# infraheads/tvidz

Hardware: AMD Instinct MI355X
Metric: 1080p frames/sec scene-cut scoring (luma SAD + select), frames resident in HBM (higher is better)
Workload: dtype u8

## Files before the change

include/tvz.h:

```cpp
#ifndef TVZ_H
#define TVZ_H

#include <stddef.h>
#include <stdint.h>

#ifdef __cplusplus
extern "C" {
#endif

#define TVZ_VERSION 403

typedef enum tvz_status {
    TVZ_OK = 0,
    TVZ_ERR_INVALID = -1,
    TVZ_ERR_HIP = -2,
    TVZ_ERR_NOMEM = -3,
    TVZ_ERR_UNSUPPORTED = -4,
    TVZ_ERR_WORKSPACE = -5,
    TVZ_ERR_COMM = -6
} tvz_status;

#define TVZ_KTH_NEVER 0x7fffffff

int tvz_version(void);
const char *tvz_last_error(void);


size_t tvz_scene_workspace_bytes(int64_t T, int32_t H, int32_t W);

size_t tvz_scene_state_bytes(int32_t H, int32_t W, int32_t bytes_per_sample);
int tvz_scene_state_reset(void *d_state, void *hip_stream);

#define TVZ_SHAPE_AUTO 0u
#define TVZ_SHAPE_NO_NT (1u << 30)
#define TVZ_SHAPE(U, tc) ((uint32_t)(U) | ((uint32_t)(tc) << 8))

int tvz_luma_sad_u8(const uint8_t *d_luma, int64_t T, int32_t H, int32_t W,
                    int64_t frame_stride_bytes, int64_t row_stride_bytes,
                    uint64_t *d_sad_out, void *d_workspace, size_t workspace_bytes,
                    void *hip_stream);

int tvz_scene_select(const uint64_t *d_sad, int64_t T, int32_t H, int32_t W,
                     int32_t bitdepth, double threshold, const double *d_prev_mafd,
                     uint8_t *d_selected, double *d_score, double *d_mafd, void *hip_stream);

int tvz_scene_scores_u8(const uint8_t *d_luma, int64_t T, int32_t H, int32_t W,
                        int64_t frame_stride_bytes, int64_t row_stride_bytes, void *d_state,
                        int32_t bitdepth, double threshold, uint64_t *d_sad_out, double *d_mafd,
                        double *d_score, uint8_t *d_selected, int32_t *d_cuts, int32_t cuts_cap,
                        void *d_workspace, size_t workspace_bytes, uint32_t shape,
                        void *hip_stream);

int tvz_scene_scores_u16(const uint16_t *d_luma, int64_t T, int32_t H, int32_t W,
                         int64_t frame_stride_bytes, int64_t row_stride_bytes, void *d_state,
                         int32_t bitdepth, double threshold, uint64_t *d_sad_out, double *d_mafd,
                         double *d_score, uint8_t *d_selected, int32_t *d_cuts, int32_t cuts_cap,
                         void *d_workspace, size_t workspace_bytes, uint32_t shape,
                         void *hip_stream);

typedef struct tvz_corpus tvz_corpus;

int tvz_corpus_create(tvz_corpus **out, int device);
int tvz_corpus_destroy(tvz_corpus *c);

int tvz_corpus_reserve(tvz_corpus *c, int64_t n_rows, int64_t n_keys);

int tvz_corpus_upload(tvz_corpus *c, const int32_t *h_video_ids, const int64_t *h_offsets,
                      const double *h_keys, int64_t n_rows, int64_t n_keys);

int tvz_corpus_upsert(tvz_corpus *c, int32_t video_id, const double *h_keys, int64_t n);

int tvz_corpus_clear(tvz_corpus *c);

int tvz_corpus_stats(tvz_corpus *c, int64_t *n_rows, int64_t *n_keys, int64_t *arena_keys);

int tvz_corpus_build_index(tvz_corpus *c);
int tvz_corpus_index_stats(tvz_corpus *c, int64_t *n_indexed_rows, int64_t *n_delta_rows,
                           int64_t *n_postings, int64_t *n_distinct_keys, int64_t *n_builds);
int tvz_corpus_bucket_stats(tvz_corpus *c, int64_t out[6]);


#define TVZ_ALGO_AUTO 0
#define TVZ_ALGO_Q1 1
#define TVZ_ALGO_TILE 2
#define TVZ_ALGO_JOIN 3
#define TVZ_ALGO_INDEX 4
#define TVZ_ALGO_PAIR 0x100
#define TVZ_ALGO_NO_PAIR 0x200
#define TVZ_ALGO_WAVE 0x400
#define TVZ_ALGO_NO_WAVE 0x800
#define TVZ_ALGO_PREFER_WAVE 0x1000

size_t tvz_match_workspace_bytes(int32_t Q, int32_t max_query_len, int32_t cap, int32_t k,
                                 int32_t n_ranks);
size_t tvz_match_workspace_bytes_long(int32_t Q, int32_t max_query_len, int32_t cap, int32_t k,
                                      int32_t n_ranks, int64_t total_query_keys);

int tvz_match(tvz_corpus *c, const double *d_queries, const int64_t *d_q_offsets,
              int32_t Q, int32_t max_query_len, int32_t min_match,
              const int32_t *d_exclude_ids, int32_t cap,
              int32_t *d_hits, int32_t *d_hits_n, void *d_workspace, size_t workspace_bytes,
              int32_t algo, void *hip_stream);

int tvz_match_topk(tvz_corpus *c, const double *d_queries, const int64_t *d_q_offsets,
                   int32_t Q, int32_t max_query_len, int32_t min_match,
                   const int32_t *d_exclude_ids, int32_t cap, int32_t k, int32_t *d_out,
                   void *d_workspace, size_t workspace_bytes, int32_t algo, void *hip_stream);

int tvz_find_duplicates(tvz_corpus *c, const double *h_query, int64_t n, int32_t min_match,
                        int32_t exclude_id, int64_t cap, int32_t *h_out_ids,
                        int32_t *h_out_counts, int32_t *h_out_kth, int64_t *n_out);

int tvz_topk(const int32_t *d_lists, const int32_t *d_lists_n, int32_t n_lists, int32_t Q,
             int32_t cap, int32_t k, int32_t *d_topk, void *hip_stream);

int tvz_topk_shard(const int32_t *d_hits, const int32_t *d_hits_n, int32_t Q, int32_t cap,
                   int32_t k, int32_t *d_out, void *hip_stream);
int tvz_match_topk_shards(tvz_corpus *const *shards, int32_t n_shards, const double *d_queries,
                          const int64_t *d_q_offsets, int32_t Q, int32_t max_query_len, int32_t min_match,
                          const int32_t *d_exclude_ids, int32_t cap, int32_t k, int32_t *d_blocks,
                          int32_t *d_topk, int32_t *d_totals, void *d_workspace, size_t workspace_bytes,
                          int32_t algo, void *hip_stream);
int tvz_topk_merge(const int32_t *d_gathered, int32_t n_ranks, int32_t Q, int32_t k,
                   int32_t *d_topk, int32_t *d_totals, void *hip_stream);

#define TVZ_UNIQUE_ID_BYTES 128
typedef struct tvz_comm tvz_comm;

int tvz_comm_unique_id(void *out_id );
int tvz_comm_init(tvz_comm **out, const void *unique_id, int32_t n_ranks, int32_t rank,
                  int32_t device);
int tvz_comm_info(tvz_comm *comm, int32_t *n_ranks, int32_t *rank);
int tvz_comm_destroy(tvz_comm *comm);

int tvz_match_sharded(tvz_corpus *c, tvz_comm *comm, const double *d_queries,
                      const int64_t *d_q_offsets, int32_t Q, int32_t max_query_len,
                      int32_t min_match, const int32_t *d_exclude_ids, int32_t cap, int32_t k,
                      int32_t *d_topk, int32_t *d_totals, void *d_workspace,
                      size_t workspace_bytes, int32_t algo, void *hip_stream);

int tvz_align(tvz_corpus *c, const double *d_query, int32_t n, double eps, double max_offset,
              int32_t *d_out, int64_t out_rows, int64_t *n_rows, void *hip_stream);


int tvz_find_duplicates_tol(tvz_corpus *c, const double *h_query, int64_t n, double tol,
                            int32_t min_match, int32_t exclude_id, int64_t cap, int32_t *h_out_ids,
                            int32_t *h_out_counts, int32_t *h_out_kth, int64_t *n_out);
size_t tvz_match_tol_workspace_bytes(int32_t Q, int32_t max_query_len, int64_t total_query_keys);
int tvz_match_tol(tvz_corpus *c, const double *d_queries, const int64_t *d_q_offsets, int32_t Q,
                  int32_t max_query_len, double tol, int32_t min_match, const int32_t *d_exclude_ids,
                  int32_t cap, int32_t *d_hits, int32_t *d_hits_n, void *d_workspace,
                  size_t workspace_bytes, void *hip_stream);

size_t tvz_match_tol_topk_workspace_bytes(int32_t Q, int32_t max_query_len, int64_t total_query_keys,
                                          int32_t k, int32_t n_ranks);
int tvz_match_tol_topk(tvz_corpus *c, const double *d_queries, const int64_t *d_q_offsets, int32_t Q,
                       int32_t max_query_len, double tol, int32_t min_match, const int32_t *d_exclude_ids,
                       int32_t k, int32_t *d_out, void *d_workspace, size_t workspace_bytes,
                       void *hip_stream);
int tvz_match_tol_sharded(tvz_corpus *c, tvz_comm *comm, const double *d_queries, const int64_t *d_q_offsets,
                          int32_t Q, int32_t max_query_len, double tol, int32_t min_match,
                          const int32_t *d_exclude_ids, int32_t k, int32_t *d_topk, int32_t *d_totals,
                          void *d_workspace, size_t workspace_bytes, void *hip_stream);


int tvz_read_records(int fd, int64_t file_offset, int64_t n_records, int64_t record_bytes,
                     const void *magic, int64_t header_bytes, int64_t payload_bytes, void *h_dst,
                     int64_t *n_done);

int tvz_read_stream(int fd, int64_t n_records, int64_t payload_bytes, int64_t skip_bytes, void *h_dst,
                    int64_t *n_done);

#ifdef __cplusplus
}
#endif
#endif
```

profiles/microbatch_scene.py:

```python
#!/usr/bin/env python3
import json
import os
import sys
import time

import numpy as np
import torch

sys.path.insert(0, os.path.dirname(os.path.dirname(os.path.abspath(__file__))))
from tvidz_amd import _lib, scene

H, W = (int(sys.argv[1]), int(sys.argv[2])) if len(sys.argv) > 2 else (1080, 1920)
dev = torch.device("cuda:0")
lib = _lib.load()
big = torch.randint(0, 256, (2048, H, W), dtype=torch.uint8, device=dev)
for T in (32, 64, 128, 256, 512, 1024, 2048):
    frames = big[:T]
    res = {}
    variants = [("auto", (0, 0, 1))] + [(f"U{u}tc{tc}", (u, tc, 1)) for u in (1, 2, 4, 8) for tc in (8, 16, 32, 64, 128, 256)]
    for name, tune in variants:
        sc = scene.SceneScorer(H, W, T, dev)
        ts = []
        for r in range(30):
            a, b = torch.cuda.Event(enable_timing=True), torch.cuda.Event(enable_timing=True)
            a.record(); sc.score_batch(frames, carry=False, shape=_lib.shape(*tune)); b.record()
            torch.cuda.synchronize()
            ts.append(a.elapsed_time(b))
        res[name] = round(float(np.median(ts[5:])) * 1e3, 1)
    best = min(res, key=res.get)
    print(json.dumps({"T": T, "auto_us": res["auto"], "best": best, "best_us": res[best],
                      "best_GBps": round((T - 1) * H * W / res[best] / 1e3, 1),
                      "top": sorted(res.items(), key=lambda kv: kv[1])[:5]}))

T = 256
host = [torch.randint(0, 256, (T, H, W), dtype=torch.uint8).pin_memory() for _ in range(2)]
devb = [torch.empty((T, H, W), dtype=torch.uint8, device=dev) for _ in range(2)]
sc = scene.SceneScorer(H, W, T, dev)
copy_s = torch.cuda.Stream()
n_batches = 40
torch.cuda.synchronize()
t0 = time.perf_counter()
evs = [None, None]
for i in range(n_batches):
    s = i & 1
    with torch.cuda.stream(copy_s):
        if evs[s] is not None:
            copy_s.wait_event(evs[s])
        devb[s].copy_(host[s], non_blocking=True)
        ce = torch.cuda.Event(); ce.record(copy_s)
    torch.cuda.current_stream().wait_event(ce)
    sc.score_batch(devb[s], carry=False)
    evs[s] = torch.cuda.Event(); evs[s].record()
torch.cuda.synchronize()
dt = time.perf_counter() - t0
print(json.dumps({"pcie_inclusive_fps": round(n_batches * T / dt), "GBps_h2d": round(n_batches * T * H * W / dt / 1e9, 1),
                  "batch": T, "note": "pinned host luma -> H2D -> score, double buffered"}))
```

profiles/tune_scene.py:

```python
#!/usr/bin/env python3
import itertools
import json
import os
import sys

import numpy as np
import torch

sys.path.insert(0, os.path.dirname(os.path.dirname(os.path.abspath(__file__))))
from tvidz_amd import _lib, scene

T = int(sys.argv[1]) if len(sys.argv) > 1 else 10000
ROUNDS = int(sys.argv[2]) if len(sys.argv) > 2 else 7
H, W = 1080, 1920
dev = torch.device("cuda:0")
lib = _lib.load()
frames = torch.randint(0, 256, (T, H, W), dtype=torch.uint8, device=dev)
if len(sys.argv) > 3 and sys.argv[3] == "tc":
    variants = [(8, tc, 1) for tc in (128, 192, 256, 320, 384, 448, 512, 640, 832, 1280, 2560)]
else:
    variants = [(U, tc, nt) for U, tc, nt in itertools.product((1, 2, 4, 8), (64, 128, 256, 512), (0, 1))]
sc = scene.SceneScorer(H, W, T, dev)
times = {v: [] for v in variants}
ref = None
for r in range(ROUNDS):
    for v in variants:
        a, b = torch.cuda.Event(enable_timing=True), torch.cuda.Event(enable_timing=True)
        a.record()
        sad, _, _, _ = sc.score_batch(frames, carry=False, shape=_lib.shape(*v))
        b.record()
        torch.cuda.synchronize()
        if r == 0:
            s = sad.clone()
            if ref is None:
                ref = s
            assert torch.equal(ref, s), v
        else:
            times[v].append(a.elapsed_time(b))
rows = []
for v, t in times.items():
    med, mn = float(np.median(t)), float(np.min(t))
    rows.append({"U": v[0], "tc": v[1], "nt": v[2], "median_ms": round(med, 4), "min_ms": round(mn, 4),
                 "GBps_median": round((T - 1) * H * W / med / 1e6, 1)})
rows.sort(key=lambda r: r["median_ms"])
for r in rows:
    print(json.dumps(r))
```

tvidz_amd/_lib.py:

```python
from __future__ import annotations

import ctypes as C
import os
import threading

_HERE = os.path.dirname(os.path.abspath(__file__))
SO_PATH = os.environ.get("TVZ_LIB") or os.path.join(_HERE, "libtvz.so")

KTH_NEVER = 0x7FFFFFFF
VERSION = 403

_P = C.c_void_p
SIGNATURES = {
    "tvz_version": (C.c_int, []),
    "tvz_last_error": (C.c_char_p, []),
    "tvz_scene_workspace_bytes": (C.c_size_t, [C.c_int64, C.c_int32, C.c_int32]),
    "tvz_scene_state_bytes": (C.c_size_t, [C.c_int32, C.c_int32, C.c_int32]),
    "tvz_scene_state_reset": (C.c_int, [_P, _P]),
    "tvz_luma_sad_u8": (C.c_int, [_P, C.c_int64, C.c_int32, C.c_int32, C.c_int64, C.c_int64,
                                  _P, _P, C.c_size_t, _P]),
    "tvz_scene_select": (C.c_int, [_P, C.c_int64, C.c_int32, C.c_int32, C.c_int32, C.c_double, _P,
                                   _P, _P, _P, _P]),
    "tvz_scene_scores_u8": (C.c_int, [_P, C.c_int64, C.c_int32, C.c_int32, C.c_int64, C.c_int64, _P,
                                      C.c_int32, C.c_double, _P, _P, _P, _P, _P, C.c_int32, _P,
                                      C.c_size_t, C.c_uint32, _P]),
    "tvz_scene_scores_u16": (C.c_int, [_P, C.c_int64, C.c_int32, C.c_int32, C.c_int64, C.c_int64, _P,
                                       C.c_int32, C.c_double, _P, _P, _P, _P, _P, C.c_int32, _P,
                                       C.c_size_t, C.c_uint32, _P]),
    "tvz_corpus_create": (C.c_int, [C.POINTER(C.c_void_p), C.c_int]),
    "tvz_corpus_destroy": (C.c_int, [_P]),
    "tvz_corpus_reserve": (C.c_int, [_P, C.c_int64, C.c_int64]),
    "tvz_corpus_upload": (C.c_int, [_P, _P, _P, _P, C.c_int64, C.c_int64]),
    "tvz_corpus_upsert": (C.c_int, [_P, C.c_int32, _P, C.c_int64]),
    "tvz_corpus_clear": (C.c_int, [_P]),
    "tvz_corpus_build_index": (C.c_int, [_P]),
    "tvz_corpus_index_stats": (C.c_int, [_P] + [C.POINTER(C.c_int64)] * 5),
    "tvz_corpus_bucket_stats": (C.c_int, [_P, C.POINTER(C.c_int64)]),
    "tvz_corpus_stats": (C.c_int, [_P, C.POINTER(C.c_int64), C.POINTER(C.c_int64),
                                   C.POINTER(C.c_int64)]),
    "tvz_match_workspace_bytes": (C.c_size_t, [C.c_int32, C.c_int32, C.c_int32, C.c_int32, C.c_int32]),
    "tvz_match_workspace_bytes_long": (C.c_size_t, [C.c_int32, C.c_int32, C.c_int32, C.c_int32, C.c_int32, C.c_int64]),
    "tvz_match": (C.c_int, [_P, _P, _P, C.c_int32, C.c_int32, C.c_int32, _P, C.c_int32, _P, _P, _P,
                            C.c_size_t, C.c_int32, _P]),
    "tvz_match_topk": (C.c_int, [_P, _P, _P, C.c_int32, C.c_int32, C.c_int32, _P, C.c_int32, C.c_int32,
                                 _P, _P, C.c_size_t, C.c_int32, _P]),
    "tvz_find_duplicates": (C.c_int, [_P, _P, C.c_int64, C.c_int32, C.c_int32, C.c_int64, _P, _P, _P,
                                      C.POINTER(C.c_int64)]),
    "tvz_topk": (C.c_int, [_P, _P, C.c_int32, C.c_int32, C.c_int32, C.c_int32, _P, _P]),
    "tvz_topk_shard": (C.c_int, [_P, _P, C.c_int32, C.c_int32, C.c_int32, _P, _P]),
    "tvz_topk_merge": (C.c_int, [_P, C.c_int32, C.c_int32, C.c_int32, _P, _P, _P]),
    "tvz_match_topk_shards": (C.c_int, [_P, C.c_int32, _P, _P, C.c_int32, C.c_int32, C.c_int32, _P, C.c_int32,
                                        C.c_int32, _P, _P, _P, _P, C.c_size_t, C.c_int32, _P]),
    "tvz_comm_unique_id": (C.c_int, [_P]),
    "tvz_comm_init": (C.c_int, [C.POINTER(C.c_void_p), _P, C.c_int32, C.c_int32, C.c_int32]),
    "tvz_comm_info": (C.c_int, [_P, C.POINTER(C.c_int32), C.POINTER(C.c_int32)]),
    "tvz_comm_destroy": (C.c_int, [_P]),
    "tvz_match_sharded": (C.c_int, [_P, _P, _P, _P, C.c_int32, C.c_int32, C.c_int32, _P, C.c_int32,
                                    C.c_int32, _P, _P, _P, C.c_size_t, C.c_int32, _P]),
    "tvz_find_duplicates_tol": (C.c_int, [_P, _P, C.c_int64, C.c_double, C.c_int32, C.c_int32, C.c_int64, _P, _P, _P,
                                          C.POINTER(C.c_int64)]),
    "tvz_match_tol_workspace_bytes": (C.c_size_t, [C.c_int32, C.c_int32, C.c_int64]),
    "tvz_match_tol": (C.c_int, [_P, _P, _P, C.c_int32, C.c_int32, C.c_double, C.c_int32, _P, C.c_int32, _P, _P, _P,
                                C.c_size_t, _P]),
    "tvz_match_tol_topk_workspace_bytes": (C.c_size_t, [C.c_int32, C.c_int32, C.c_int64, C.c_int32, C.c_int32]),
    "tvz_match_tol_topk": (C.c_int, [_P, _P, _P, C.c_int32, C.c_int32, C.c_double, C.c_int32, _P, C.c_int32, _P, _P,
                                     C.c_size_t, _P]),
    "tvz_match_tol_sharded": (C.c_int, [_P, _P, _P, _P, C.c_int32, C.c_int32, C.c_double, C.c_int32, _P, C.c_int32,
                                        _P, _P, _P, C.c_size_t, _P]),
    "tvz_align": (C.c_int, [_P, _P, C.c_int32, C.c_double, C.c_double, _P, C.c_int64, C.POINTER(C.c_int64), _P]),
    "tvz_read_records": (C.c_int, [C.c_int, C.c_int64, C.c_int64, C.c_int64, _P, C.c_int64, C.c_int64, _P,
                                   C.POINTER(C.c_int64)]),
    "tvz_read_stream": (C.c_int, [C.c_int, C.c_int64, C.c_int64, C.c_int64, _P, C.POINTER(C.c_int64)]),
}

ALGO_AUTO, ALGO_Q1, ALGO_TILE, ALGO_JOIN, ALGO_INDEX = 0, 1, 2, 3, 4
ALGO_PAIR, ALGO_NO_PAIR = 0x100, 0x200
ALGO_WAVE, ALGO_NO_WAVE = 0x400, 0x800
ALGO_PREFER_WAVE = 0x1000
SHAPE_AUTO = 0
SHAPE_NO_NT = 1 << 30
UNIQUE_ID_BYTES = 128


def shape(U: int = 0, tc: int = 0, nt: bool = True) -> int:
    s = (int(U) & 0xFF) | (int(tc) << 8)
    if not nt:
        s |= SHAPE_NO_NT
    return s


_lock = threading.Lock()
_lib = None


def _preload_torch_hip_runtime() -> None:
    import torch
    cand = os.path.join(os.path.dirname(torch.__file__), "lib", "libamdhip64.so")
    if os.path.exists(cand):
        C.CDLL(cand, mode=C.RTLD_GLOBAL)


def load() -> C.CDLL:
    global _lib
    if _lib is not None:
        return _lib
    with _lock:
        if _lib is None:
            if not os.path.exists(SO_PATH):
                raise RuntimeError(
                    f"{SO_PATH} is missing: the HIP extension is not built and there is no CPU "
                    "fallback. Run `python -m tvidz_amd.build` (needs hipcc).")
            _preload_torch_hip_runtime()
            lib = C.CDLL(SO_PATH)
            lib.tvz_version.restype, lib.tvz_version.argtypes = C.c_int, []
            if lib.tvz_version() == -VERSION and os.environ.get("TVZ_ALLOW_DIAGNOSTIC") != "1":
                raise RuntimeError(f"{SO_PATH} is a DIAGNOSTIC build (tvz_version() = {lib.tvz_version()}: compiled with "
                                   "a TVZ_IX_* / TVZ_DIAGNOSTIC define; some of them return wrong results on purpose). "
                                   "The product binding refuses it; profile scripts set TVZ_ALLOW_DIAGNOSTIC=1.")
            if abs(lib.tvz_version()) != VERSION:
                raise RuntimeError(f"{SO_PATH} is version {lib.tvz_version()}, this binding expects {VERSION}: "
                                   "rebuild it (python -m tvidz_amd.build --force)")
            for name, (res, args) in SIGNATURES.items():
                fn = getattr(lib, name)
                fn.restype = res
                fn.argtypes = args
            _lib = lib
    return _lib


def check(rc: int) -> None:
    if rc != 0:
        msg = load().tvz_last_error()
        raise RuntimeError(f"libtvz error {rc}: {(msg or b'').decode(errors='replace')}")
```

tvidz_amd/csrc/tvz_scene.hip:

```cpp
#include <algorithm>

#include "tvz_common.h"

namespace {

constexpr int kWave = 64;
#ifndef TVZ_SCENE_BLOCK
#define TVZ_SCENE_BLOCK 256
#endif
constexpr int kBlock = TVZ_SCENE_BLOCK;
constexpr int kWavesPerBlock = kBlock / kWave;

struct Tuning {
    int U = 0;
    int tc = 0;
    int nt = 1;
};

struct StateHdr {
    double prev_mafd;
    int32_t have_prev;
    int32_t parity;
    int64_t frames_seen;
};
constexpr size_t kStateHdrBytes = 256;
struct WsHdr {
    double last_mafd;
};
constexpr size_t kWsHdrBytes = 256;

struct StateArgs {
    StateHdr *hdr;
    uint8_t *buf0, *buf1;
};

struct Carry {
    const uint8_t *prev0;
    uint8_t *tail;
    int32_t t_first;
};
__device__ __forceinline__ Carry read_carry(const StateArgs &sa) {
    Carry c{nullptr, nullptr, 1};
    if (sa.hdr) {
        const int32_t have = sa.hdr->have_prev, par = sa.hdr->parity;
        c.prev0 = par ? sa.buf1 : sa.buf0;
        c.tail = par ? sa.buf0 : sa.buf1;
        c.t_first = have ? 0 : 1;
    }
    return c;
}

template <int CTRL, int ROW_MASK>
__device__ __forceinline__ uint32_t dpp_add(uint32_t v) {
    return v + (uint32_t)__builtin_amdgcn_update_dpp(0, (int)v, CTRL, ROW_MASK, 0xf, false);
}

__device__ __forceinline__ uint32_t wave_sum_u32(uint32_t v) {
    v = dpp_add<0x111, 0xf>(v);
    v = dpp_add<0x112, 0xf>(v);
    v = dpp_add<0x114, 0xf>(v);
    v = dpp_add<0x118, 0xf>(v);
    v = dpp_add<0x142, 0xa>(v);
    v = dpp_add<0x143, 0xc>(v);
    return (uint32_t)__builtin_amdgcn_readlane((int)v, 63);
}

template <bool S16>
__device__ __forceinline__ uint32_t sad_dword(uint32_t a, uint32_t b, uint32_t acc) {
    if constexpr (S16) return __builtin_amdgcn_sad_u16(a, b, acc);
    else return __builtin_amdgcn_sad_u8(a, b, acc);
}

template <bool S16>
__device__ __forceinline__ uint32_t sad16(const uint4 &a, const uint4 &b, uint32_t acc) {
    acc = sad_dword<S16>(a.x, b.x, acc);
    acc = sad_dword<S16>(a.y, b.y, acc);
    acc = sad_dword<S16>(a.z, b.z, acc);
    acc = sad_dword<S16>(a.w, b.w, acc);
    return acc;
}

struct Stash {
    uint32_t v = 0;
    __device__ __forceinline__ void put(int lane, int64_t t, uint32_t total) {
        if (lane == (int)(t & 63)) v = total;
    }
    __device__ __forceinline__ void maybe_flush(int lane, int64_t t, int64_t t_lo, int64_t t_last,
                                                uint32_t *__restrict__ row) {
        if ((t & 63) == 63 || t == t_last) {
            const int64_t tb = t & ~(int64_t)63;
            const int64_t lt = tb + lane;
            if (lt >= t_lo && lt <= t) row[lt] = v;
        }
    }
};

template <bool NT>
__device__ __forceinline__ uint4 load16(const uint4 *p) {
    if constexpr (NT) {
        using v4 = __attribute__((ext_vector_type(4))) unsigned int;
        const v4 v = __builtin_nontemporal_load(reinterpret_cast<const v4 *>(p));
        return make_uint4(v.x, v.y, v.z, v.w);
    } else {
        return *p;
    }
}

template <int U, bool NT, bool S16>
__global__ __launch_bounds__(kBlock) void luma_sad_flat_kernel(
    const uint8_t *__restrict__ luma, StateArgs sa, int64_t T, int64_t frame_stride, int64_t n16,
    int32_t n_strips, int32_t tc, uint32_t *__restrict__ partial, int64_t Tpad) {
    const int lane = threadIdx.x & 63;
    const int strip = blockIdx.x * kWavesPerBlock + (threadIdx.x >> 6);
    if (strip >= n_strips) return;
    const Carry cy = read_carry(sa);
    int64_t t0 = (int64_t)blockIdx.y * tc;
    const int64_t t1 = (t0 + tc < T) ? t0 + tc : T;
    if (t0 < cy.t_first) t0 = cy.t_first;
    const bool keep_tail = cy.tail != nullptr && t1 == T;

    int64_t idx[U];
    bool ok[U];
#pragma unroll
    for (int u = 0; u < U; ++u) {
        const int64_t i = ((int64_t)strip * U + u) * kWave + lane;
        ok[u] = i < n16;
        idx[u] = ok[u] ? i : 0;
    }
    uint4 prev[U], cur[U], nxt[U];
    if (t0 >= t1) {
        if (keep_tail) {
            const uint4 *pl = reinterpret_cast<const uint4 *>(luma + (T - 1) * frame_stride);
            uint4 *pt = reinterpret_cast<uint4 *>(cy.tail);
#pragma unroll
            for (int u = 0; u < U; ++u)
                if (ok[u]) pt[idx[u]] = load16<NT>(pl + idx[u]);
        }
        return;
    }
    const uint4 *pp = (t0 == 0) ? reinterpret_cast<const uint4 *>(cy.prev0)
                                : reinterpret_cast<const uint4 *>(luma + (t0 - 1) * frame_stride);
    const uint4 *pc = reinterpret_cast<const uint4 *>(luma + t0 * frame_stride);
#pragma unroll
    for (int u = 0; u < U; ++u) prev[u] = load16<NT>(pp + idx[u]);
#pragma unroll
    for (int u = 0; u < U; ++u) cur[u] = load16<NT>(pc + idx[u]);

    uint32_t *row = partial + (int64_t)strip * Tpad;
    Stash stash;
    auto score = [&](int64_t t) {
        uint32_t acc = 0;
#pragma unroll
        for (int u = 0; u < U; ++u) {
            const uint32_t a = sad16<S16>(cur[u], prev[u], acc);
            acc = ok[u] ? a : acc;
        }
        const uint32_t total = wave_sum_u32(acc);
        stash.put(lane, t, total);
        stash.maybe_flush(lane, t, t0, t1 - 1, row);
    };
    for (int64_t t = t0; t < t1 - 1; ++t) {
        const uint4 *pn = reinterpret_cast<const uint4 *>(luma + (t + 1) * frame_stride);
#pragma unroll
        for (int u = 0; u < U; ++u) nxt[u] = load16<NT>(pn + idx[u]);
        score(t);
#pragma unroll
        for (int u = 0; u < U; ++u) {
            prev[u] = cur[u];
            cur[u] = nxt[u];
        }
    }
    score(t1 - 1);
    if (keep_tail) {
        uint4 *pt = reinterpret_cast<uint4 *>(cy.tail);
#pragma unroll
        for (int u = 0; u < U; ++u)
            if (ok[u]) pt[idx[u]] = cur[u];
    }
}

__device__ __forceinline__ uint32_t load_granule(const uint8_t *p, int nb) {
    uint32_t v = 0;
    if (nb == 4) {
        __builtin_memcpy(&v, p, 4);
    } else {
        for (int i = 0; i < nb; ++i) v |= (uint32_t)p[i] << (8 * i);
    }
    return v;
}

__device__ __forceinline__ void store_granule(uint8_t *p, uint32_t v, int nb) {
    if (nb == 4) {
        __builtin_memcpy(p, &v, 4);
    } else {
        for (int i = 0; i < nb; ++i) p[i] = (uint8_t)(v >> (8 * i));
    }
}

template <int U, bool S16>
__global__ __launch_bounds__(kBlock) void luma_sad_generic_kernel(
    const uint8_t *__restrict__ luma, StateArgs sa, int64_t T, int64_t frame_stride,
    int64_t row_stride, int32_t H, int32_t W , int32_t gpr, int64_t n_gran,
    int32_t n_strips, int32_t tc, uint32_t *__restrict__ partial, int64_t Tpad) {
    const int lane = threadIdx.x & 63;
    const int strip = blockIdx.x * kWavesPerBlock + (threadIdx.x >> 6);
    if (strip >= n_strips) return;
    const Carry cy = read_carry(sa);
    int64_t t0 = (int64_t)blockIdx.y * tc;
    const int64_t t1 = (t0 + tc < T) ? t0 + tc : T;
    if (t0 < cy.t_first) t0 = cy.t_first;
    const bool keep_tail = cy.tail != nullptr && t1 == T;

    int64_t off[U], off0[U];
    int nb[U];
#pragma unroll
    for (int u = 0; u < U; ++u) {
        const int64_t g = ((int64_t)strip * U + u) * kWave + lane;
        if (g < n_gran) {
            const int64_t y = g / gpr;
            const int32_t x = (int32_t)(g - y * gpr) * 4;
            nb[u] = (W - x < 4) ? (W - x) : 4;
            off[u] = y * row_stride + x;
            off0[u] = y * (int64_t)W + x;
        } else {
            nb[u] = 0;
            off[u] = 0;
            off0[u] = 0;
        }
    }
    uint32_t prev[U], cur[U];
    if (t0 >= t1) {
        if (keep_tail) {
#pragma unroll
            for (int u = 0; u < U; ++u)
                store_granule(cy.tail + off0[u], load_granule(luma + (T - 1) * frame_stride + off[u], nb[u]), nb[u]);
        }
        return;
    }
#pragma unroll
    for (int u = 0; u < U; ++u)
        prev[u] = (t0 == 0) ? load_granule(cy.prev0 + off0[u], nb[u])
                            : load_granule(luma + (t0 - 1) * frame_stride + off[u], nb[u]);
    uint32_t *row = partial + (int64_t)strip * Tpad;
    Stash stash;
    for (int64_t t = t0; t < t1; ++t) {
        const uint8_t *pc = luma + t * frame_stride;
        uint32_t acc = 0;
#pragma unroll
        for (int u = 0; u < U; ++u) {
            cur[u] = load_granule(pc + off[u], nb[u]);
            acc = sad_dword<S16>(cur[u], prev[u], acc);
            prev[u] = cur[u];
        }
        const uint32_t total = wave_sum_u32(acc);
        stash.put(lane, t, total);
        stash.maybe_flush(lane, t, t0, t1 - 1, row);
    }
    if (keep_tail) {
#pragma unroll
        for (int u = 0; u < U; ++u) store_granule(cy.tail + off0[u], prev[u], nb[u]);
    }
}

struct SelectParams {
    double count;
    double depth_div;
    double threshold;
};

__device__ __forceinline__ double mafd_of(uint64_t sad, const SelectParams &p) {
    return (double)sad / p.count / p.depth_div;
}

__device__ __forceinline__ void scene_epilogue(uint64_t sad, bool first, double prev_mafd,
                                               const SelectParams &p, double &mafd, double &score,
                                               uint8_t &sel) {
    if (first) {
        mafd = 0.0;
        score = 0.0;
        sel = 0;
        return;
    }
    mafd = mafd_of(sad, p);
    const double diff = fabs(mafd - prev_mafd);
    const double m = (mafd > diff) ? diff : mafd;
    float f = (float)(m / 100.);
    f = (f < 0.0f) ? 0.0f : ((f > 1.0f) ? 1.0f : f);
    score = (double)f;
    sel = (score > p.threshold) ? 1 : 0;
}

constexpr int kFinT = 64;
constexpr int kFinG = 16;

__global__ __launch_bounds__(kFinT *kFinG) void scene_finalize_kernel(
    const uint32_t *__restrict__ partial, int32_t n_strips, int64_t Tpad, int64_t T,
    const StateHdr *__restrict__ st, SelectParams sp, uint64_t *__restrict__ sad_out,
    double *__restrict__ mafd_out, double *__restrict__ score_out, uint8_t *__restrict__ sel_out,
    WsHdr *__restrict__ wh) {
    __shared__ uint64_t red[kFinG][kFinT + 1];
    int32_t t_first = 1;
    double prev_mafd_in = 0.0;
    if (st && st->have_prev) {
        t_first = 0;
        prev_mafd_in = st->prev_mafd;
    }
    const int tl = threadIdx.x & (kFinT - 1);
    const int sg = threadIdx.x / kFinT;
    const int64_t bt = (int64_t)blockIdx.x * kFinT;
    const int64_t t = bt + tl;
    uint64_t acc = 0, halo = 0;
    if (t < T && t >= t_first)
        for (int s = sg; s < n_strips; s += kFinG) acc += partial[(int64_t)s * Tpad + t];
    if (tl == 0 && bt - 1 >= t_first)
        for (int s = sg; s < n_strips; s += kFinG) halo += partial[(int64_t)s * Tpad + bt - 1];
    red[sg][tl] = acc;
    if (tl == 0) red[sg][kFinT] = halo;
    __syncthreads();
    if (threadIdx.x <= kFinT) {
        uint64_t s = 0;
#pragma unroll
        for (int g = 0; g < kFinG; ++g) s += red[g][threadIdx.x];
        red[0][threadIdx.x] = s;
    }
    __syncthreads();
    if (sg == 0 && t < T) {
        const uint64_t sad = red[0][tl];
        if (sad_out) sad_out[t] = sad;
        const bool first = t < t_first;
        double prev_mafd = prev_mafd_in;
        if (t - 1 >= t_first) prev_mafd = mafd_of(tl ? red[0][tl - 1] : red[0][kFinT], sp);
        double mafd, score;
        uint8_t sel;
        scene_epilogue(sad, first, prev_mafd, sp, mafd, score, sel);
        if (mafd_out) mafd_out[t] = mafd;
        if (score_out) score_out[t] = score;
        if (sel_out) sel_out[t] = sel;
        if (t == T - 1) wh->last_mafd = mafd;
    }
}

__global__ __launch_bounds__(256) void scene_select_kernel(const uint64_t *__restrict__ sad,
                                                           int64_t T,
                                                           const double *__restrict__ d_prev_mafd,
                                                           SelectParams sp,
                                                           uint8_t *__restrict__ sel_out,
                                                           double *__restrict__ score_out,
                                                           double *__restrict__ mafd_out) {
    const int64_t t = (int64_t)blockIdx.x * blockDim.x + threadIdx.x;
    if (t >= T) return;
    const int64_t t_first = d_prev_mafd ? 0 : 1;
    double prev_mafd = d_prev_mafd ? *d_prev_mafd : 0.0;
    if (t - 1 >= t_first) prev_mafd = mafd_of(sad[t - 1], sp);
    double mafd, score;
    uint8_t sel;
    scene_epilogue(sad[t], t < t_first, prev_mafd, sp, mafd, score, sel);
    sel_out[t] = sel;
    if (score_out) score_out[t] = score;
    if (mafd_out) mafd_out[t] = mafd;
}

constexpr int kTailBlock = 1024;
__global__ __launch_bounds__(kTailBlock) void scene_tail_kernel(
    const uint8_t *__restrict__ sel, int64_t T, int32_t *__restrict__ cuts, int32_t cuts_cap,
    StateHdr *__restrict__ st, const WsHdr *__restrict__ wh) {
    __shared__ int32_t wsum[kTailBlock / 64];
    const int lane = threadIdx.x & 63, wave = threadIdx.x >> 6;
    if (cuts) {
        const int64_t c = (T + kTailBlock - 1) / kTailBlock;
        const int64_t t0 = (int64_t)threadIdx.x * c;
        const int64_t t1 = t0 + c < T ? t0 + c : T;
        int mine = 0;
        for (int64_t t = t0; t < t1; ++t) mine += sel[t] != 0;
        int incl = mine;
#pragma unroll
        for (int off = 1; off < 64; off <<= 1) {
            const int v = __shfl_up(incl, off);
            if (lane >= off) incl += v;
        }
        if (lane == 63) wsum[wave] = incl;
        __syncthreads();
        int base = 0, total = 0;
        for (int w = 0; w < kTailBlock / 64; ++w) {
            const int v = wsum[w];
            if (w < wave) base += v;
            total += v;
        }
        int pos = base + incl - mine;
        for (int64_t t = t0; t < t1; ++t)
            if (sel[t] != 0) {
                if (pos < cuts_cap) cuts[1 + pos] = (int32_t)t;
                ++pos;
            }
        if (threadIdx.x == 0) cuts[0] = total;
    }
    if (st && threadIdx.x == 0) {
        st->prev_mafd = wh->last_mafd;
        st->have_prev = 1;
        st->parity ^= 1;
        st->frames_seen += T;
    }
}

__global__ void scene_state_reset_kernel(StateHdr *st) {
    st->prev_mafd = 0.0;
    st->have_prev = 0;
    st->parity = 0;
    st->frames_seen = 0;
}

struct Plan {
    bool flat;
    int U;
    int tc;
    int64_t n16;
    int64_t n_gran;
    int32_t gpr;
    int32_t n_strips;
    int64_t Tpad;
};

constexpr int kGenericU = 8;

bool flat_ok(const void *p, int64_t fs, int64_t rs, int32_t H, int32_t W, int bps) {
    return rs == (int64_t)W * bps && ((int64_t)H * W * bps) % 16 == 0 && fs % 16 == 0 &&
           (reinterpret_cast<uintptr_t>(p) % 16) == 0;
}

void auto_shape(int64_t T, int64_t n16, int &U, int &tc) {
    U = 8;
    const int64_t strips = tvz::ceil_div(n16, (int64_t)kWave * U);
    const int64_t chunks = std::max<int64_t>(1, 1024 / std::max<int64_t>(1, strips));
    const int64_t want = tvz::ceil_div(T, chunks);
    tc = 8;
    while (tc < 256 && tc < want) tc *= 2;
}

int decode_shape(uint32_t shape, Tuning &tn) {
    tn = Tuning{};
    if (shape == TVZ_SHAPE_AUTO) return TVZ_OK;
    tn.nt = (shape & TVZ_SHAPE_NO_NT) ? 0 : 1;
    tn.U = (int)(shape & 0xffu);
    tn.tc = (int)((shape >> 8) & 0xfffffu);
    TVZ_REQUIRE(tn.U == 0 || tn.U == 1 || tn.U == 2 || tn.U == 4 || tn.U == 8,
                "shape: U must be 0 (auto), 1, 2, 4 or 8");
    TVZ_REQUIRE(tn.tc == 0 || tn.tc == 8 || tn.tc == 16 || tn.tc == 32 || tn.tc % 64 == 0,
                "shape: tc must be 0 (auto), 8, 16, 32 or a multiple of 64");
    return TVZ_OK;
}

Plan make_plan(bool flat, int64_t T, int32_t H, int32_t W, int bps, const Tuning &tn) {
    Plan p{};
    p.flat = flat;
    p.tc = tn.tc ? tn.tc : 128;
    p.Tpad = tvz::round_up(T > 0 ? T : 1, 64);
    if (flat) {
        p.n16 = (int64_t)H * W * bps / 16;
        int aU = 4, atc = 128;
        auto_shape(T > 0 ? T : 1, p.n16, aU, atc);
        p.U = tn.U ? tn.U : aU;
        p.tc = tn.tc ? tn.tc : atc;
        p.n_strips = (int32_t)tvz::ceil_div(p.n16, (int64_t)kWave * p.U);
    } else {
        p.U = kGenericU;
        p.gpr = (W * bps + 3) / 4;
        p.n_gran = (int64_t)H * p.gpr;
        p.n_strips = (int32_t)tvz::ceil_div(p.n_gran, (int64_t)kWave * p.U);
    }
    return p;
}

size_t plan_bytes(const Plan &p) { return (size_t)p.n_strips * (size_t)p.Tpad * sizeof(uint32_t); }

int check_dims(int64_t T, int32_t H, int32_t W) {
    TVZ_REQUIRE(T >= 0, "T must be >= 0 (got %lld)", (long long)T);
    TVZ_REQUIRE(H > 0 && W > 0, "H and W must be positive (got %d x %d)", H, W);
    if ((int64_t)H * W > (int64_t)1 << 31)
        return tvz::fail(TVZ_ERR_UNSUPPORTED, "frame of %d x %d exceeds 2^31 pixels", H, W);
    return TVZ_OK;
}

size_t state_frame_bytes(int32_t H, int32_t W, int bps) {
    return (size_t)tvz::round_up((int64_t)H * W * bps, 256);
}

int launch_sad(const uint8_t *d_luma, const StateArgs &sa, int64_t T, int32_t H, int32_t W,
               int64_t fs, int64_t rs, const Plan &p, uint32_t *partial, int bps, int nt,
               hipStream_t st) {
    dim3 grid((unsigned)tvz::ceil_div(p.n_strips, kWavesPerBlock), (unsigned)tvz::ceil_div(T, p.tc));
    if (grid.y > 65535u)
        return tvz::fail(TVZ_ERR_UNSUPPORTED, "batch of %lld frames needs more than 65535 time chunks",
                         (long long)T);
    if (p.flat) {
#define TVZ_FLAT_(UU, NTV, S16V)                                                               \
    hipLaunchKernelGGL((luma_sad_flat_kernel<UU, NTV, S16V>), grid, dim3(kBlock), 0, st, d_luma,   \
                       sa, T, fs, p.n16, p.n_strips, p.tc, partial, p.Tpad)
#define TVZ_FLAT(UU)                                                                           \
    do {                                                                                       \
        if (bps == 2) { if (nt) TVZ_FLAT_(UU, true, true); else TVZ_FLAT_(UU, false, true); }   \
        else          { if (nt) TVZ_FLAT_(UU, true, false); else TVZ_FLAT_(UU, false, false); } \
    } while (0)
        switch (p.U) {
            case 1: TVZ_FLAT(1); break;
            case 2: TVZ_FLAT(2); break;
            case 4: TVZ_FLAT(4); break;
            case 8: TVZ_FLAT(8); break;
            default: return tvz::fail(TVZ_ERR_INVALID, "unsupported U=%d", p.U);
        }
#undef TVZ_FLAT
#undef TVZ_FLAT_
    } else {
        if (bps == 2)
            hipLaunchKernelGGL((luma_sad_generic_kernel<kGenericU, true>), grid, dim3(kBlock), 0, st,
                               d_luma, sa, T, fs, rs, H, W * 2, p.gpr, p.n_gran, p.n_strips,
                               p.tc, partial, p.Tpad);
        else
            hipLaunchKernelGGL((luma_sad_generic_kernel<kGenericU, false>), grid, dim3(kBlock), 0, st,
                               d_luma, sa, T, fs, rs, H, W, p.gpr, p.n_gran, p.n_strips, p.tc,
                               partial, p.Tpad);
    }
    TVZ_HIP(hipGetLastError());
    return TVZ_OK;
}

SelectParams make_sp(int32_t H, int32_t W, int32_t bitdepth, double thr) {
    SelectParams sp;
    sp.count = (double)((uint64_t)W * (uint64_t)H);
    sp.depth_div = (double)(1ULL << (bitdepth - 8));
    sp.threshold = thr;
    return sp;
}

}

TVZ_EXPORT size_t tvz_scene_workspace_bytes(int64_t T, int32_t H, int32_t W) {
    if (T < 0 || H <= 0 || W <= 0) return 0;
    const size_t a = (size_t)tvz::ceil_div((int64_t)H * W * 2 / 16 + 1, kWave) * (size_t)tvz::round_up(T > 0 ? T : 1, 64) * sizeof(uint32_t);
    const size_t b = plan_bytes(make_plan(false, T, H, W, 2, Tuning{}));
    return (a > b ? a : b) + kWsHdrBytes + 256;
}

TVZ_EXPORT size_t tvz_scene_state_bytes(int32_t H, int32_t W, int32_t bytes_per_sample) {
    if (H <= 0 || W <= 0 || (bytes_per_sample != 1 && bytes_per_sample != 2)) return 0;
    return kStateHdrBytes + 2 * state_frame_bytes(H, W, bytes_per_sample);
}

TVZ_EXPORT int tvz_scene_state_reset(void *d_state, void *hip_stream) {
    TVZ_REQUIRE(d_state != nullptr, "d_state is NULL");
    TVZ_REQUIRE(reinterpret_cast<uintptr_t>(d_state) % 256 == 0, "d_state must be 256-byte aligned");
    hipLaunchKernelGGL(scene_state_reset_kernel, dim3(1), dim3(1), 0,
                       reinterpret_cast<hipStream_t>(hip_stream), reinterpret_cast<StateHdr *>(d_state));
    TVZ_HIP(hipGetLastError());
    return TVZ_OK;
}

namespace {
int scene_scores_impl(const uint8_t *d_luma, int bps, int64_t T, int32_t H, int32_t W,
                      int64_t frame_stride_bytes, int64_t row_stride_bytes, void *d_state,
                      int32_t bitdepth, double threshold, uint64_t *d_sad_out, double *d_mafd,
                      double *d_score, uint8_t *d_selected, int32_t *d_cuts, int32_t cuts_cap,
                      void *d_workspace, size_t workspace_bytes, uint32_t shape, void *hip_stream) {
    if (int rc = check_dims(T, H, W)) return rc;
    if (T == 0) return TVZ_OK;
    TVZ_REQUIRE(d_luma != nullptr, "d_luma is NULL");
    TVZ_REQUIRE(row_stride_bytes >= (int64_t)W * bps, "row stride %lld < %d bytes",
                (long long)row_stride_bytes, W * bps);
    TVZ_REQUIRE(frame_stride_bytes >= (int64_t)(H - 1) * row_stride_bytes + (int64_t)W * bps || T == 1,
                "frame stride %lld smaller than a plane", (long long)frame_stride_bytes);
    if (bps == 1) TVZ_REQUIRE(bitdepth == 8, "8-bit entry point called with bitdepth=%d", bitdepth);
    else {
        TVZ_REQUIRE(bitdepth > 8 && bitdepth <= 16, "16-bit entry point needs 9 <= bitdepth <= 16 (got %d)", bitdepth);
        TVZ_REQUIRE(row_stride_bytes % 2 == 0 && frame_stride_bytes % 2 == 0 &&
                        reinterpret_cast<uintptr_t>(d_luma) % 2 == 0,
                    "16-bit planes must be 2-byte aligned");
    }
    TVZ_REQUIRE(d_sad_out || d_selected || d_score || d_mafd || d_state,
                "nothing to compute: every output is NULL");
    TVZ_REQUIRE(d_cuts == nullptr || (d_selected != nullptr && cuts_cap >= 0),
                "d_cuts needs d_selected and cuts_cap >= 0");
    TVZ_REQUIRE(d_workspace != nullptr, "d_workspace is NULL");
    TVZ_REQUIRE(d_state == nullptr || reinterpret_cast<uintptr_t>(d_state) % 256 == 0,
                "d_state must be 256-byte aligned");
    Tuning tn;
    if (int rc = decode_shape(shape, tn)) return rc;
    hipStream_t st = reinterpret_cast<hipStream_t>(hip_stream);
    const bool flat = flat_ok(d_luma, frame_stride_bytes, row_stride_bytes, H, W, bps);
    const Plan p = make_plan(flat, T, H, W, bps, tn);
    uintptr_t ws = (reinterpret_cast<uintptr_t>(d_workspace) + 255) & ~(uintptr_t)255;
    const size_t lost = ws - reinterpret_cast<uintptr_t>(d_workspace);
    if (workspace_bytes < lost + kWsHdrBytes + plan_bytes(p))
        return tvz::fail(TVZ_ERR_WORKSPACE, "workspace of %zu bytes, need %zu", workspace_bytes,
                         lost + kWsHdrBytes + plan_bytes(p));
    WsHdr *wh = reinterpret_cast<WsHdr *>(ws);
    uint32_t *partial = reinterpret_cast<uint32_t *>(ws + kWsHdrBytes);
    StateArgs sa{nullptr, nullptr, nullptr};
    if (d_state) {
        sa.hdr = reinterpret_cast<StateHdr *>(d_state);
        sa.buf0 = reinterpret_cast<uint8_t *>(d_state) + kStateHdrBytes;
        sa.buf1 = sa.buf0 + state_frame_bytes(H, W, bps);
    }
    if (int rc = launch_sad(d_luma, sa, T, H, W, frame_stride_bytes, row_stride_bytes, p, partial,
                            bps, tn.nt, st))
        return rc;
    const SelectParams sp = make_sp(H, W, bitdepth, threshold);
    hipLaunchKernelGGL(scene_finalize_kernel, dim3((unsigned)tvz::ceil_div(T, kFinT)),
                       dim3(kFinT * kFinG), 0, st, partial, p.n_strips, p.Tpad, T, sa.hdr, sp,
                       d_sad_out, d_mafd, d_score, d_selected, wh);
    TVZ_HIP(hipGetLastError());
    if (d_cuts || d_state) {
        hipLaunchKernelGGL(scene_tail_kernel, dim3(1), dim3(kTailBlock), 0, st, d_selected, T, d_cuts,
                           cuts_cap, sa.hdr, wh);
        TVZ_HIP(hipGetLastError());
    }
    return TVZ_OK;
}
}

TVZ_EXPORT int tvz_scene_scores_u8(const uint8_t *d_luma, int64_t T, int32_t H, int32_t W,
                                   int64_t frame_stride_bytes, int64_t row_stride_bytes,
                                   void *d_state, int32_t bitdepth, double threshold,
                                   uint64_t *d_sad_out, double *d_mafd, double *d_score,
                                   uint8_t *d_selected, int32_t *d_cuts, int32_t cuts_cap,
                                   void *d_workspace, size_t workspace_bytes, uint32_t shape,
                                   void *hip_stream) {
    return scene_scores_impl(d_luma, 1, T, H, W, frame_stride_bytes, row_stride_bytes, d_state,
                             bitdepth, threshold, d_sad_out, d_mafd, d_score, d_selected, d_cuts,
                             cuts_cap, d_workspace, workspace_bytes, shape, hip_stream);
}

TVZ_EXPORT int tvz_scene_scores_u16(const uint16_t *d_luma, int64_t T, int32_t H, int32_t W,
                                    int64_t frame_stride_bytes, int64_t row_stride_bytes,
                                    void *d_state, int32_t bitdepth, double threshold,
                                    uint64_t *d_sad_out, double *d_mafd, double *d_score,
                                    uint8_t *d_selected, int32_t *d_cuts, int32_t cuts_cap,
                                    void *d_workspace, size_t workspace_bytes, uint32_t shape,
                                    void *hip_stream) {
    return scene_scores_impl(reinterpret_cast<const uint8_t *>(d_luma), 2, T, H, W,
                             frame_stride_bytes, row_stride_bytes, d_state, bitdepth, threshold,
                             d_sad_out, d_mafd, d_score, d_selected, d_cuts, cuts_cap, d_workspace,
                             workspace_bytes, shape, hip_stream);
}

TVZ_EXPORT int tvz_luma_sad_u8(const uint8_t *d_luma, int64_t T, int32_t H, int32_t W,
                               int64_t frame_stride_bytes, int64_t row_stride_bytes,
                               uint64_t *d_sad_out, void *d_workspace, size_t workspace_bytes,
                               void *hip_stream) {
    TVZ_REQUIRE(d_sad_out != nullptr || T == 0, "d_sad_out is NULL");
    return tvz_scene_scores_u8(d_luma, T, H, W, frame_stride_bytes, row_stride_bytes, nullptr, 8,
                               0.0, d_sad_out, nullptr, nullptr, nullptr, nullptr, 0, d_workspace,
                               workspace_bytes, TVZ_SHAPE_AUTO, hip_stream);
}

TVZ_EXPORT int tvz_scene_select(const uint64_t *d_sad, int64_t T, int32_t H, int32_t W,
                                int32_t bitdepth, double threshold, const double *d_prev_mafd,
                                uint8_t *d_selected, double *d_score, double *d_mafd,
                                void *hip_stream) {
    if (int rc = check_dims(T, H, W)) return rc;
    if (T == 0) return TVZ_OK;
    TVZ_REQUIRE(d_sad && d_selected, "d_sad / d_selected is NULL");
    TVZ_REQUIRE(bitdepth >= 8 && bitdepth <= 16, "bitdepth %d out of range", bitdepth);
    const SelectParams sp = make_sp(H, W, bitdepth, threshold);
    hipLaunchKernelGGL(scene_select_kernel, dim3((unsigned)tvz::ceil_div(T, 256)), dim3(256), 0,
                       reinterpret_cast<hipStream_t>(hip_stream), d_sad, T, d_prev_mafd, sp,
                       d_selected, d_score, d_mafd);
    TVZ_HIP(hipGetLastError());
    return TVZ_OK;
}
```

Before: 3.221 million.

## Add configurable multi-frame prefetch ring to flat luma SAD kernel

Replaces the prev/cur/next register rotation in the flat SAD kernel with an N-slot register ring that keeps D frames of loads in flight, paced by explicit waitcnt and sched barriers. Loads now take a scalar frame base plus a 32-bit per-lane offset instead of 64-bit indices, which cuts address arithmetic. A depth field is added to the shape encoding and launch-bounds occupancy hints scale with depth. Auto shape still picks D=1, so the default path only gains the new addressing, pacing and unrolled loop structure, while deeper rings raise register pressure.

```diff
diff --git a/include/tvz.h b/include/tvz.h
--- a/include/tvz.h
+++ b/include/tvz.h
@@ -34,6 +34,7 @@
 #define TVZ_SHAPE_AUTO 0u
 #define TVZ_SHAPE_NO_NT (1u << 30)
 #define TVZ_SHAPE(U, tc) ((uint32_t)(U) | ((uint32_t)(tc) << 8))
+#define TVZ_SHAPE_DEPTH(D) ((uint32_t)((D) == 1 ? 1u : (D) == 2 ? 2u : (D) == 4 ? 3u : 0u) << 28)
 
 int tvz_luma_sad_u8(const uint8_t *d_luma, int64_t T, int32_t H, int32_t W,
                     int64_t frame_stride_bytes, int64_t row_stride_bytes,
diff --git a/profiles/microbatch_scene.py b/profiles/microbatch_scene.py
--- a/profiles/microbatch_scene.py
+++ b/profiles/microbatch_scene.py
@@ -18,6 +18,7 @@
     frames = big[:T]
     res = {}
     variants = [("auto", (0, 0, 1))] + [(f"U{u}tc{tc}", (u, tc, 1)) for u in (1, 2, 4, 8) for tc in (8, 16, 32, 64, 128, 256)]
+    variants += [(f"U8tc{tc}D{d}", (8, tc, 1, d)) for tc in (64, 128, 256, 512) for d in (2, 4)]
     for name, tune in variants:
         sc = scene.SceneScorer(H, W, T, dev)
         ts = []
diff --git a/profiles/tune_scene.py b/profiles/tune_scene.py
--- a/profiles/tune_scene.py
+++ b/profiles/tune_scene.py
@@ -18,6 +18,9 @@
 frames = torch.randint(0, 256, (T, H, W), dtype=torch.uint8, device=dev)
 if len(sys.argv) > 3 and sys.argv[3] == "tc":
     variants = [(8, tc, 1) for tc in (128, 192, 256, 320, 384, 448, 512, 640, 832, 1280, 2560)]
+elif len(sys.argv) > 3 and sys.argv[3] == "ring":
+    tcs = [int(x) for x in sys.argv[4].split(",")] if len(sys.argv) > 4 else (256, 640, 1280, 1728, 2560, 5056)
+    variants = [(0, 0, 1, 0)] + [(8, tc, 1, D) for tc in tcs for D in (1, 2, 4)]
 else:
     variants = [(U, tc, nt) for U, tc, nt in itertools.product((1, 2, 4, 8), (64, 128, 256, 512), (0, 1))]
 sc = scene.SceneScorer(H, W, T, dev)
@@ -40,7 +43,8 @@
 rows = []
 for v, t in times.items():
     med, mn = float(np.median(t)), float(np.min(t))
-    rows.append({"U": v[0], "tc": v[1], "nt": v[2], "median_ms": round(med, 4), "min_ms": round(mn, 4),
+    rows.append({"U": v[0], "tc": v[1], "nt": v[2], **({"D": v[3], "chunks": -(-T // v[1]) if v[1] else "auto"} if len(v) > 3 else {}),
+                 "median_ms": round(med, 4), "min_ms": round(mn, 4),
                  "GBps_median": round((T - 1) * H * W / med / 1e6, 1)})
 rows.sort(key=lambda r: r["median_ms"])
 for r in rows:
diff --git a/tvidz_amd/_lib.py b/tvidz_amd/_lib.py
--- a/tvidz_amd/_lib.py
+++ b/tvidz_amd/_lib.py
@@ -82,8 +82,10 @@
 UNIQUE_ID_BYTES = 128
 
 
-def shape(U: int = 0, tc: int = 0, nt: bool = True) -> int:
-    s = (int(U) & 0xFF) | (int(tc) << 8)
+def shape(U: int = 0, tc: int = 0, nt: bool = True, D: int = 0) -> int:
+    if int(D) not in (0, 1, 2, 4):
+        raise ValueError(f"shape: D must be 0 (auto), 1, 2 or 4 (got {D})")
+    s = (int(U) & 0xFF) | (int(tc) << 8) | ({0: 0, 1: 1, 2: 2, 4: 3}[int(D)] << 28)
     if not nt:
         s |= SHAPE_NO_NT
     return s
diff --git a/tvidz_amd/csrc/tvz_scene.hip b/tvidz_amd/csrc/tvz_scene.hip
--- a/tvidz_amd/csrc/tvz_scene.hip
+++ b/tvidz_amd/csrc/tvz_scene.hip
@@ -15,6 +15,7 @@
     int U = 0;
     int tc = 0;
     int nt = 1;
+    int D = 0;
 };
 
 struct StateHdr {
@@ -96,20 +97,23 @@
 };
 
 template <bool NT>
-__device__ __forceinline__ uint4 load16(const uint4 *p) {
-    if constexpr (NT) {
-        using v4 = __attribute__((ext_vector_type(4))) unsigned int;
-        const v4 v = __builtin_nontemporal_load(reinterpret_cast<const v4 *>(p));
-        return make_uint4(v.x, v.y, v.z, v.w);
-    } else {
-        return *p;
-    }
-}
-
-template <int U, bool NT, bool S16>
-__global__ __launch_bounds__(kBlock) void luma_sad_flat_kernel(
+__device__ __forceinline__ uint4 load16(const uint8_t *frame, uint32_t off) {
+    using v4 = __attribute__((ext_vector_type(4))) unsigned int;
+    using gv4 = const __attribute__((address_space(1))) v4;
+    uint64_t base = reinterpret_cast<uint64_t>(frame);
+    asm("" : "+s"(base));
+    gv4 *p = (gv4 *)(base + off);
+    const v4 v = NT ? __builtin_nontemporal_load(p) : *p;
+    return make_uint4(v.x, v.y, v.z, v.w);
+}
+
+constexpr int flat_waves_per_simd(int D) { return D <= 1 ? 4 : D == 2 ? 3 : 2; }
+
+template <int U, bool NT, bool S16, int D>
+__global__ __launch_bounds__(kBlock, flat_waves_per_simd(D)) void luma_sad_flat_kernel(
     const uint8_t *__restrict__ luma, StateArgs sa, int64_t T, int64_t frame_stride, int64_t n16,
     int32_t n_strips, int32_t tc, uint32_t *__restrict__ partial, int64_t Tpad) {
+    constexpr int N = D + 2;
     const int lane = threadIdx.x & 63;
     const int strip = blockIdx.x * kWavesPerBlock + (threadIdx.x >> 6);
     if (strip >= n_strips) return;
@@ -119,63 +123,86 @@
     if (t0 < cy.t_first) t0 = cy.t_first;
     const bool keep_tail = cy.tail != nullptr && t1 == T;
 
-    int64_t idx[U];
+    uint32_t off[U];
     bool ok[U];
 #pragma unroll
     for (int u = 0; u < U; ++u) {
         const int64_t i = ((int64_t)strip * U + u) * kWave + lane;
         ok[u] = i < n16;
-        idx[u] = ok[u] ? i : 0;
-    }
-    uint4 prev[U], cur[U], nxt[U];
+        off[u] = ok[u] ? (uint32_t)(i * 16) : 0u;
+    }
     if (t0 >= t1) {
         if (keep_tail) {
-            const uint4 *pl = reinterpret_cast<const uint4 *>(luma + (T - 1) * frame_stride);
-            uint4 *pt = reinterpret_cast<uint4 *>(cy.tail);
+            const uint8_t *pl = luma + (T - 1) * frame_stride;
 #pragma unroll
             for (int u = 0; u < U; ++u)
-                if (ok[u]) pt[idx[u]] = load16<NT>(pl + idx[u]);
+                if (ok[u]) *reinterpret_cast<uint4 *>(cy.tail + off[u]) = load16<NT>(pl, off[u]);
         }
         return;
     }
-    const uint4 *pp = (t0 == 0) ? reinterpret_cast<const uint4 *>(cy.prev0)
-                                : reinterpret_cast<const uint4 *>(luma + (t0 - 1) * frame_stride);
-    const uint4 *pc = reinterpret_cast<const uint4 *>(luma + t0 * frame_stride);
-#pragma unroll
-    for (int u = 0; u < U; ++u) prev[u] = load16<NT>(pp + idx[u]);
-#pragma unroll
-    for (int u = 0; u < U; ++u) cur[u] = load16<NT>(pc + idx[u]);
-
+    const int64_t n = t1 - t0;
+    const uint8_t *f0 = luma + t0 * frame_stride;
+    uint4 ring[N][U];
+    auto pace = [] {
+        constexpr int c = (D - 1) * U;
+        __builtin_amdgcn_sched_barrier(0);
+        __builtin_amdgcn_s_waitcnt((c & 0xf) | ((c >> 4) << 14) | 0x0f70);
+    };
+    auto issue = [&](int slot, const uint8_t *frame) {
+#pragma unroll
+        for (int u = 0; u < U; ++u) ring[slot][u] = load16<NT>(frame, off[u]);
+        __builtin_amdgcn_sched_barrier(0);
+    };
     uint32_t *row = partial + (int64_t)strip * Tpad;
     Stash stash;
-    auto score = [&](int64_t t) {
+    auto score = [&](int cur, int prev, int64_t t) {
         uint32_t acc = 0;
 #pragma unroll
         for (int u = 0; u < U; ++u) {
-            const uint32_t a = sad16<S16>(cur[u], prev[u], acc);
+            const uint32_t a = sad16<S16>(ring[cur][u], ring[prev][u], acc);
             acc = ok[u] ? a : acc;
         }
         const uint32_t total = wave_sum_u32(acc);
         stash.put(lane, t, total);
         stash.maybe_flush(lane, t, t0, t1 - 1, row);
     };
-    for (int64_t t = t0; t < t1 - 1; ++t) {
-        const uint4 *pn = reinterpret_cast<const uint4 *>(luma + (t + 1) * frame_stride);
-#pragma unroll
-        for (int u = 0; u < U; ++u) nxt[u] = load16<NT>(pn + idx[u]);
-        score(t);
-#pragma unroll
-        for (int u = 0; u < U; ++u) {
-            prev[u] = cur[u];
-            cur[u] = nxt[u];
-        }
-    }
-    score(t1 - 1);
-    if (keep_tail) {
-        uint4 *pt = reinterpret_cast<uint4 *>(cy.tail);
-#pragma unroll
-        for (int u = 0; u < U; ++u)
-            if (ok[u]) pt[idx[u]] = cur[u];
+    const uint8_t *pp = (t0 == 0) ? cy.prev0 : f0 - frame_stride;
+    int64_t k = 0;
+    if (n >= N + D) {
+        issue(0, pp);
+        issue(1, f0);
+#pragma unroll
+        for (int d = 1; d < D; ++d) issue(d + 1, f0 + d * frame_stride);
+        do {
+#pragma unroll
+            for (int j = 0; j < N; ++j) {
+                pace();
+                issue((j + D + 1) % N, f0 + (k + j + D) * frame_stride);
+                score((j + 1) % N, j % N, t0 + k + j);
+            }
+            k += N;
+        } while (k + (N - 1) + D < n);
+    } else {
+        issue(0, pp);
+        issue(1, f0);
+#pragma unroll
+        for (int d = 1; d < D; ++d)
+            if (d < n) issue(d + 1, f0 + d * frame_stride);
+    }
+#pragma unroll
+    for (int j = 0; j < N - 1 + D; ++j) {
+        if (k + j < n) {
+            if (k + j + D < n) {
+                pace();
+                issue((j + D + 1) % N, f0 + (k + j + D) * frame_stride);
+            }
+            score((j + 1) % N, j % N, t0 + k + j);
+            if (keep_tail && k + j == n - 1) {
+#pragma unroll
+                for (int u = 0; u < U; ++u)
+                    if (ok[u]) *reinterpret_cast<uint4 *>(cy.tail + off[u]) = ring[(j + 1) % N][u];
+            }
+        }
     }
 }
 
@@ -413,6 +440,7 @@
     bool flat;
     int U;
     int tc;
+    int D;
     int64_t n16;
     int64_t n_gran;
     int32_t gpr;
@@ -427,13 +455,14 @@
            (reinterpret_cast<uintptr_t>(p) % 16) == 0;
 }
 
-void auto_shape(int64_t T, int64_t n16, int &U, int &tc) {
+void auto_shape(int64_t T, int64_t n16, int &U, int &tc, int &D) {
     U = 8;
     const int64_t strips = tvz::ceil_div(n16, (int64_t)kWave * U);
     const int64_t chunks = std::max<int64_t>(1, 1024 / std::max<int64_t>(1, strips));
     const int64_t want = tvz::ceil_div(T, chunks);
     tc = 8;
     while (tc < 256 && tc < want) tc *= 2;
+    D = 1;
 }
 
 int decode_shape(uint32_t shape, Tuning &tn) {
@@ -442,10 +471,13 @@
     tn.nt = (shape & TVZ_SHAPE_NO_NT) ? 0 : 1;
     tn.U = (int)(shape & 0xffu);
     tn.tc = (int)((shape >> 8) & 0xfffffu);
+    const int dcode = (int)((shape >> 28) & 3u);
+    tn.D = dcode ? 1 << (dcode - 1) : 0;
     TVZ_REQUIRE(tn.U == 0 || tn.U == 1 || tn.U == 2 || tn.U == 4 || tn.U == 8,
                 "shape: U must be 0 (auto), 1, 2, 4 or 8");
     TVZ_REQUIRE(tn.tc == 0 || tn.tc == 8 || tn.tc == 16 || tn.tc == 32 || tn.tc % 64 == 0,
                 "shape: tc must be 0 (auto), 8, 16, 32 or a multiple of 64");
+    TVZ_REQUIRE(tn.D <= 1 || tn.U == 0 || tn.U == 8, "shape: a depth above 1 needs U = 8 (or 0, auto)");
     return TVZ_OK;
 }
 
@@ -456,10 +488,11 @@
     p.Tpad = tvz::round_up(T > 0 ? T : 1, 64);
     if (flat) {
         p.n16 = (int64_t)H * W * bps / 16;
-        int aU = 4, atc = 128;
-        auto_shape(T > 0 ? T : 1, p.n16, aU, atc);
+        int aU = 8, atc = 128, aD = 1;
+        auto_shape(T > 0 ? T : 1, p.n16, aU, atc, aD);
         p.U = tn.U ? tn.U : aU;
         p.tc = tn.tc ? tn.tc : atc;
+        p.D = tn.D ? tn.D : (p.U == 8 ? aD : 1);
         p.n_strips = (int32_t)tvz::ceil_div(p.n16, (int64_t)kWave * p.U);
     } else {
         p.U = kGenericU;
@@ -492,20 +525,22 @@
         return tvz::fail(TVZ_ERR_UNSUPPORTED, "batch of %lld frames needs more than 65535 time chunks",
                          (long long)T);
     if (p.flat) {
-#define TVZ_FLAT_(UU, NTV, S16V)                                                               \
-    hipLaunchKernelGGL((luma_sad_flat_kernel<UU, NTV, S16V>), grid, dim3(kBlock), 0, st, d_luma,   \
+#define TVZ_FLAT_(UU, NTV, S16V, DD)                                                            \
+    hipLaunchKernelGGL((luma_sad_flat_kernel<UU, NTV, S16V, DD>), grid, dim3(kBlock), 0, st, d_luma, \
                        sa, T, fs, p.n16, p.n_strips, p.tc, partial, p.Tpad)
-#define TVZ_FLAT(UU)                                                                           \
+#define TVZ_FLAT(UU, DD)                                                                       \
     do {                                                                                       \
-        if (bps == 2) { if (nt) TVZ_FLAT_(UU, true, true); else TVZ_FLAT_(UU, false, true); }   \
-        else          { if (nt) TVZ_FLAT_(UU, true, false); else TVZ_FLAT_(UU, false, false); } \
+        if (bps == 2) { if (nt) TVZ_FLAT_(UU, true, true, DD); else TVZ_FLAT_(UU, false, true, DD); }   \
+        else          { if (nt) TVZ_FLAT_(UU, true, false, DD); else TVZ_FLAT_(UU, false, false, DD); } \
     } while (0)
-        switch (p.U) {
-            case 1: TVZ_FLAT(1); break;
-            case 2: TVZ_FLAT(2); break;
-            case 4: TVZ_FLAT(4); break;
-            case 8: TVZ_FLAT(8); break;
-            default: return tvz::fail(TVZ_ERR_INVALID, "unsupported U=%d", p.U);
+        switch (p.U * 8 + p.D) {
+            case 1 * 8 + 1: TVZ_FLAT(1, 1); break;
+            case 2 * 8 + 1: TVZ_FLAT(2, 1); break;
+            case 4 * 8 + 1: TVZ_FLAT(4, 1); break;
+            case 8 * 8 + 1: TVZ_FLAT(8, 1); break;
+            case 8 * 8 + 2: TVZ_FLAT(8, 2); break;
+            case 8 * 8 + 4: TVZ_FLAT(8, 4); break;
+            default: return tvz::fail(TVZ_ERR_INVALID, "unsupported U=%d with depth %d", p.U, p.D);
         }
 #undef TVZ_FLAT
 #undef TVZ_FLAT_
```

Result: no change. 3.230 million (median of 6 runs) (+0.3%).
